# m3db/m3

Measured on AMD Instinct MI355X. Metric: datapoints/sec M3TSZ decode (1M series x 1440 pts) + HBM GB/s vs peak, higher is better.
Workload: dtype f64; 1 GPU; 1M series x 1440 pts batched M3TSZ decode, HBM-bandwidth microbench; nseries=1000000, npts=1440, data_detail=synthetic, parallelism=series-sharded x1 (no collectives)

## Files before the change

### m3_amd/csrc/m3tsz_kernels.hip

```cpp
#include <hip/hip_runtime.h>
#include <atomic>
#include <math.h>
#include <string.h>
#include <stdio.h>
#include "../../include/m3gpu.h"
#include "rollup_plan.h"


#define WAVE 64
#define WAVES_PER_BLOCK 4
#define BLOCK_THREADS (WAVE * WAVES_PER_BLOCK)

namespace m3 {

__device__ __constant__ int64_t UNIT_NS_D[9] = {
    0, 1000000000LL, 1000000LL, 1000LL, 1LL,
    60000000000LL, 3600000000000LL, 86400000000000LL, 31536000000000000LL};

#define MARKER_OPCODE 0x100ULL
#define MARKER_BITS 11
#define MARKER_EOS 0
#define MARKER_ANNOTATION 1
#define MARKER_TIMEUNIT 2

// ... 402 lines not shown
                prev_time_delta += dod;
                prev_time += prev_time_delta;
            }
        } else {
            *first = true;
            err = read_first_timestamp();
        }
        if (err) return err;
        if (tu_changed) { prev_time_delta = 0; tu_changed = false; }
        return 0;
    }

    __device__ __forceinline__ int read_full_float() {
        uint64_t vb;
        int err = r.read_bits(64, &vb);
        if (err) return err;
        prev_float_bits = vb;
        prev_xor = vb;
        return 0;
    }
    __device__ __forceinline__ int read_next_float() {
        uint64_t cb;
        int err = r.read_bits(1, &cb);
        if (err) return err;
        if (cb == 0) { prev_xor = 0; return 0; }
        uint64_t nxt;
        err = r.read_bits(1, &nxt);
        if (err) return err;
        cb = (cb << 1) | nxt;
        if (cb == 0x2) {
            uint32_t lead = prev_xor ? __builtin_clzll(prev_xor) : 64;
            uint32_t trail = prev_xor ? __builtin_ctzll(prev_xor) : 0;
            uint32_t nmean = 64 - lead - trail;
            uint64_t mb;
            err = r.read_bits(nmean, &mb);
            if (err) return err;
            prev_xor = mb << trail;
            prev_float_bits ^= prev_xor;
            return 0;
        }
        uint64_t lm;
        err = r.read_bits(12, &lm);
        if (err) return err;
        uint64_t lead = (lm & 4032) >> 6;
        uint64_t nmean = (lm & 63) + 1;
        uint64_t mb;
        err = r.read_bits((uint32_t)nmean, &mb);
        if (err) return err;
        uint64_t trail = 64 - lead - nmean;
        prev_xor = mb << trail;
        prev_float_bits ^= prev_xor;
        return 0;
    }

    __device__ __forceinline__ int read_int_sig_mult() {
        uint64_t b;
        int err = r.read_bits(1, &b);
        if (err) return err;
        if (b == 1) {
            err = r.read_bits(1, &b);
            if (err) return err;
            if (b == 0) sig = 0;
            else {
                uint64_t s;
                err = r.read_bits(NUM_SIG_BITS, &s);
                if (err) return err;
                sig = (uint8_t)s + 1;
            }
        }
        err = r.read_bits(1, &b);
        if (err) return err;
        if (b == 1) {
            uint64_t m;
            err = r.read_bits(NUM_MULT_BITS, &m);
            if (err) return err;
            mult = (uint8_t)m;
            if (mult > MAX_MULT) return M3GPU_SERIES_INVALID_MULT;
            mult_pow = exp10_sel(mult);
        }
        return 0;
    }
    __device__ __forceinline__ int read_int_val_diff() {
        if (sig == 64) {
            uint64_t sb;
            int err = r.read_bits(1, &sb);
            if (err) return err;
            double sgn = (sb == 1) ? 1.0 : -1.0;
            uint64_t bits;
            err = r.read_bits(sig, &bits);
            if (err) return err;
            int_val += sgn * (double)bits;
            return 0;
        }
        uint64_t bits;
        int err = r.read_bits((uint32_t)sig + 1, &bits);
        if (err) return err;
        double sgn = -1.0;
        if ((bits >> sig) == 1) { sgn = 1.0; bits ^= (1ULL << sig); }
        int_val += sgn * (double)bits;
        return 0;
    }

    __device__ __forceinline__ int read_first_value() {
        if (!int_optimized) return read_full_float();
        uint64_t b;
        int err = r.read_bits(1, &b);
        if (err) return err;
        if (b == 1) {
            err = read_full_float();
            if (err) return err;
            is_float = true;
            return 0;
        }
        err = read_int_sig_mult();
        if (err) return err;
        return read_int_val_diff();
    }
    __device__ __forceinline__ int read_next_value() {
        if (!int_optimized) return read_next_float();
        uint64_t b;
        int err = r.read_bits(1, &b);
        if (err) return err;
        if (b == 0) {
            err = r.read_bits(1, &b);
            if (err) return err;
            if (b == 1) return 0;
            err = r.read_bits(1, &b);
            if (err) return err;
            if (b == 1) {
                err = read_full_float();
                if (err) return err;
                is_float = true;
                return 0;
            }
            err = read_int_sig_mult();
            if (err) return err;
            err = read_int_val_diff();
            if (err) return err;
            is_float = false;
            return 0;
        }
        if (is_float) return read_next_float();
        return read_int_val_diff();
    }

    __device__ __forceinline__ int fused_xor(uint64_t w2, uint32_t pre) {
        if (!(w2 >> 63)) {
            r.consume(pre + 1);
            prev_xor = 0;
            return 0;
        }
        if ((w2 >> 62) == 0x2) {
            uint32_t lead = prev_xor ? __builtin_clzll(prev_xor) : 64;
            uint32_t trail = prev_xor ? __builtin_ctzll(prev_xor) : 0;
            uint32_t nmean = 64 - lead - trail;
            if (pre + 2 + nmean > 64) return -1000;
            uint64_t mb = nmean ? ((w2 << 2) >> (64 - nmean)) : 0;
            r.consume(pre + 2 + nmean);
            prev_xor = mb << trail;
            prev_float_bits ^= prev_xor;
            return 0;
        }
        uint64_t lead = (w2 >> 56) & 0x3f;
        uint64_t nmean = ((w2 >> 50) & 0x3f) + 1;
        r.consume(pre + 14);
        uint64_t mb;
        int err = r.read_bits((uint32_t)nmean, &mb);
        if (err) return -err;
        uint64_t trail = 64 - lead - nmean;
        prev_xor = mb << trail;
        prev_float_bits ^= prev_xor;
        return 0;
    }

    __device__ __forceinline__ int next_fused(int64_t* t, double* v) {
        if (tu_changed || !have_scheme || prev_time == 0 || r.bits_left < 64)
            return -1000;
        const uint64_t w = r.peek64();
        const uint64_t b0 = w >> 63;
        uint32_t tsbits = 1;
        int64_t dod = 0;
        if (b0) {
            const uint32_t L = (uint32_t)__builtin_clzll(~w);
            if (L >= 4 || (w >> 55) == MARKER_OPCODE)
                return -1000;
            const uint32_t vb = (0xC970u >> (L * 4)) & 0xFu;
            tsbits = L + 1 + vb;
            dod = sign_extend((w << (L + 1)) >> (64 - vb), vb) * unit_ns;
        }
        const uint64_t w2 = w << tsbits;

        if (int_optimized && !is_float) {
            const uint64_t v0 = w2 >> 63;
            const uint64_t v1 = (w2 >> 62) & 1;
            uint32_t nb;
            if (v0) {
                if (sig > 45u || tsbits + 2u + sig > 64u)
                    return -1000;
                nb = 2u + sig;
                const uint64_t field = (w2 << 1) >> (63u - sig);
                const uint64_t sbit = (field >> sig) & 1;
                const uint64_t mag = field ^ (sbit << sig);
                int_val += (sbit ? 1.0 : -1.0) * (double)mag;
            } else if (v1) {
                nb = 2;
            } else if ((w2 >> 61) & 1) {
                return -1000;
            } else {
                const uint64_t u = w2 << 3;
                uint8_t nsig = sig;
                uint32_t off;
                if (u >> 63) {
                    const uint64_t z = (u >> 62) & 1;
                    nsig = z ? (uint8_t)(((u >> 56) & 0x3f) + 1) : 0;
                    off = z ? 8u : 2u;
                } else {
                    off = 1u;
                }
                const uint64_t m = u << off;
                uint8_t nmult = mult;
                uint32_t moff;
                if (m >> 63) {
                    nmult = (uint8_t)((m >> 60) & 0x7);
                    moff = 4u;
                    if (nmult > MAX_MULT)
                        return -1000;
                } else {
                    moff = 1u;
                }
                if (nsig > 45u || tsbits + 3u + off + moff + 1u + nsig > 64u)
                    return -1000;
                const uint64_t f = m << moff;
                const uint64_t sbit = f >> 63;
                const uint64_t mag =
                    nsig ? ((f << 1) >> ((64u - nsig) & 63u)) : 0;
                int_val += (sbit ? 1.0 : -1.0) * (double)mag;
                sig = nsig;
                if (nmult != mult) { mult = nmult; mult_pow = exp10_sel(nmult); }
                nb = 3u + off + moff + 1u + nsig;
            }
            r.consume(tsbits + nb);
            prev_time_delta += dod;
            prev_time += prev_time_delta;
            *t = prev_time;
            double outv = int_val;
            if (mult != 0) outv = int_val / mult_pow;
            *v = outv;
            return 1;
        }
        int rx;
        if (!int_optimized) {
            rx = fused_xor(w2, tsbits);
        } else if (w2 >> 63) {
            rx = fused_xor(w2 << 1, tsbits + 1);
        } else if ((w2 >> 62) & 1) {
            r.consume(tsbits + 2);
            rx = 0;
        } else {
            return -1000;
        }
        if (rx == -1000) return -1000;
        if (rx) return rx;
        prev_time_delta += dod;
        prev_time += prev_time_delta;
        *t = prev_time;
        *v = bits2f(prev_float_bits);
        return 1;
    }

    __device__ __forceinline__ int next(int64_t* t, double* v) {
        if (done) return 0;
        int f = next_fused(t, v);
        if (f != -1000) {
            points += (f == 1);
            return f;
        }
        bool first;
        int err = read_timestamp(&first);
        if (err) return -err;
        if (done) return 0;
        err = first ? read_first_value() : read_next_value();
        if (err) return -err;
        *t = prev_time;
        if (!int_optimized || is_float) *v = bits2f(prev_float_bits);
        else if (mult != 0) *v = int_val / mult_pow;
        else *v = int_val;
        points++;
        return 1;
    }
    __device__ __forceinline__ double exp10_table(uint8_t m) {
        return exp10_sel(m);
    }
};

using Decoder = DecoderT<false>;
using RingDecoder = DecoderT<true>;


#define DEC_TILE 8
#ifndef RF_SPAN
#define RF_SPAN 2
#endif

__global__ void __launch_bounds__(BLOCK_THREADS, 4)
k_decode_batch(const uint8_t* __restrict__ blobs,
               const uint64_t* __restrict__ offsets,
               const uint32_t* __restrict__ lens,
               const int32_t* __restrict__ perm,
               uint32_t nseries, int int_optimized, uint8_t default_unit,
               int64_t* __restrict__ out_ts, double* __restrict__ out_vals,
               uint32_t* __restrict__ out_counts, int32_t* __restrict__ out_errs,
               uint32_t stride,
               uint8_t* __restrict__ out_ann, uint32_t ann_stride) {
    const uint32_t lane = threadIdx.x & (WAVE - 1);
    const uint32_t wave = __builtin_amdgcn_readfirstlane(threadIdx.x >> 6);
    const uint32_t slot = blockIdx.x * BLOCK_THREADS + wave * WAVE + lane;
    const uint32_t series = (perm && slot < nseries) ? (uint32_t)perm[slot] : slot;

    __shared__ uint64_t ring_all[WAVES_PER_BLOCK][WAVE][IN_STRIDE];
    __shared__ longlong2 tile_all[WAVES_PER_BLOCK][WAVE][DEC_TILE];
    uint64_t* ring = ring_all[wave][lane];
    longlong2 (*tile)[DEC_TILE] = tile_all[wave];

    const bool in_range = slot < nseries;
    RingDecoder d;
    d.init(blobs, in_range ? offsets[series] : 0, in_range ? lens[series] : 0,
           int_optimized != 0, default_unit, ring,
           (out_ann && in_range) ? out_ann + (uint64_t)series * ann_stride
                                 : nullptr,
           ann_stride);

    bool running = in_range;
    int err = 0;
    uint32_t cnt = 0;
    uint32_t k = 0;

    const bool discard = out_ts == nullptr;

    auto flush = [&](uint32_t base_pt) {
        if (discard) return;
        __builtin_amdgcn_wave_barrier();
        const uint32_t p = lane & (DEC_TILE - 1);
        const uint32_t r0 = lane / DEC_TILE;
        const uint32_t pt = base_pt + p;
        if (__all(cnt >= base_pt + DEC_TILE)) {
            for (uint32_t j = 0; j < DEC_TILE; j++) {
                uint32_t rr = r0 + j * (WAVE / DEC_TILE);
                uint32_t pc = p ^ (rr & 7);
                uint64_t row = (uint64_t)__shfl((int)series, (int)rr);
                longlong2 pr = tile[rr][pc];
                out_ts[row * stride + pt] = pr.x;
                out_vals[row * stride + pt] = __longlong_as_double(pr.y);
            }
        } else {
            for (uint32_t j = 0; j < DEC_TILE; j++) {
                uint32_t rr = r0 + j * (WAVE / DEC_TILE);
                uint32_t pc = p ^ (rr & 7);
                uint32_t cc = (uint32_t)__shfl((int)cnt, (int)rr);
                uint64_t row = (uint64_t)__shfl((int)series, (int)rr);
                if (pt < cc) {
                    longlong2 pr = tile[rr][pc];
                    out_ts[row * stride + pt] = pr.x;
                    out_vals[row * stride + pt] = __longlong_as_double(pr.y);
                }
            }
        }
        __builtin_amdgcn_wave_barrier();
    };

    auto step = [&](uint32_t j, bool check_cap) {
        if (running) {
            int64_t t;
            double v;
            int rstat = d.next(&t, &v);
            if (rstat <= 0) {
                err = -rstat;
                running = false;
            } else if (check_cap && cnt >= stride) {
                err = M3GPU_SERIES_CAPACITY;
                running = false;
            } else {
                if (!discard) {
                    uint32_t col = j ^ (lane & 7);
                    longlong2 pr;
                    pr.x = t;
                    pr.y = __double_as_longlong(v);
                    tile[lane][col] = pr;
                }
                cnt++;
            }
        }
    };

    while (__any(running)) {
        const bool check_cap = k + DEC_TILE > stride;
#pragma unroll 1
        for (uint32_t h = 0; h < DEC_TILE; h += RF_SPAN) {
            const RingPending pd = d.r.refill_issue(running);
#pragma unroll 1
            for (uint32_t j = h; j < h + RF_SPAN; j++) step(j, check_cap);
            d.r.refill_commit(pd);
        }
        flush(k);
        k += DEC_TILE;
    }

    if (in_range) {
        d.ann_finish(&err);
        out_counts[series] = cnt;
        out_errs[series] = err;
    }
}


struct BitWriter {
    uint64_t acc;
    uint32_t used;
    uint32_t nwords;
    uint64_t pend;
    uint64_t* out;
    uint32_t cap_words;
    int err;

    __device__ __forceinline__ void init(uint8_t* row, uint32_t cap_bytes) {
        acc = 0; used = 0; nwords = 0; pend = 0;
        out = (uint64_t*)row;
        cap_words = cap_bytes / 8;
        err = 0;
    }
    __device__ __forceinline__ void emit_word(uint64_t w) {
        if (nwords >= cap_words) { err = M3GPU_SERIES_CAPACITY; return; }
        if (nwords & 1) {
            ulonglong2 pr;
            pr.x = pend;
            pr.y = __builtin_bswap64(w);
            *(ulonglong2*)(out + nwords - 1) = pr;
        } else {
            pend = __builtin_bswap64(w);
        }
        nwords++;
    }
    __device__ __forceinline__ void write_bits(uint64_t v, uint32_t n) {
        if (n == 0 || err) return;
        v = (n >= 64) ? v : (v & ((1ULL << n) - 1));
        uint32_t space = 64 - used;
        if (n <= space) {
            acc |= v << (space - n);
            used += n;
            if (used == 64) { emit_word(acc); acc = 0; used = 0; }
        } else {
            uint32_t lo = n - space;
            acc |= v >> lo;
            emit_word(acc);
            acc = (lo >= 64) ? 0 : (v << (64 - lo));
            used = lo;
        }
    }
    __device__ __forceinline__ void write_bit(uint32_t b) { write_bits(b, 1); }
    __device__ __forceinline__ uint32_t finish() {
        if (nwords & 1) out[nwords - 1] = pend;
        uint32_t nbytes = nwords * 8;
        if (used > 0) {
            if (nwords >= cap_words) { err = M3GPU_SERIES_CAPACITY; return 0; }
            out[nwords] = __builtin_bswap64(acc);
            nbytes += (used + 7) / 8;
        }
        return nbytes;
    }
};

__device__ __forceinline__ double go_next_down(double x) {
    return __longlong_as_double(__double_as_longlong(x) - 1);
}
__device__ __forceinline__ double go_next_up(double x) {
    return __longlong_as_double(__double_as_longlong(x) + 1);
}

__device__ __forceinline__ int convert_to_int_float(double v, uint8_t cur_max_mult,
                                    double* out_val, uint8_t* out_mult, bool* out_is_float) {
    const double MAXINT = 9223372036854775808.0;
    if (cur_max_mult == 0 && v < MAXINT) {
        double i, r;
        r = go_modf(v, &i);
        if (r == 0) { *out_val = i; *out_mult = 0; *out_is_float = false; return 0; }
    }
    if (cur_max_mult > MAX_MULT) return M3GPU_SERIES_INVALID_MULT;
    double sign = 1.0;
    if (v < 0) sign = -1.0;
    for (uint8_t m = cur_max_mult; m <= MAX_MULT; m++) {
        double val = v * exp10_sel(m) * sign;
        if (val >= 1e13) break;
        double i, r;
        r = go_modf(val, &i);
        if (r == 0) { *out_val = sign * i; *out_mult = m; *out_is_float = false; return 0; }
        else if (r < 0.1) {
            if (go_next_down(val) <= i) { *out_val = sign * i; *out_mult = m; *out_is_float = false; return 0; }
        } else if (r > 0.9) {
            double nxt = i + 1;
            if (go_next_up(val) >= nxt) { *out_val = sign * nxt; *out_mult = m; *out_is_float = false; return 0; }
        }
    }
    *out_val = v; *out_mult = 0; *out_is_float = true;
    return 0;
}

#define XXH_P1 11400714785074694791ULL
#define XXH_P2 14029467366897019727ULL
#define XXH_P3 1609587929392839161ULL
#define XXH_P4 9650029242287828579ULL
#define XXH_P5 2870177450012600261ULL
#define XXH_EMPTY 0xEF46DB3751D8E999ULL

__device__ __forceinline__ uint64_t ld_le64(const uint8_t* p) {
    uint64_t v; __builtin_memcpy(&v, p, 8); return v;
}
__device__ __forceinline__ uint32_t ld_le32(const uint8_t* p) {
    uint32_t v; __builtin_memcpy(&v, p, 4); return v;
}
__device__ __forceinline__ uint64_t xxh_rotl(uint64_t x, uint32_t r) {
    return (x << r) | (x >> (64 - r));
}
__device__ __forceinline__ uint64_t xxh_round(uint64_t acc, uint64_t in) {
    return xxh_rotl(acc + in * XXH_P2, 31) * XXH_P1;
}
__device__ __forceinline__ uint64_t xxh_merge(uint64_t h, uint64_t v) {
    return (h ^ xxh_round(0, v)) * XXH_P1 + XXH_P4;
}
__device__ __noinline__ uint64_t xxh64(const uint8_t* p, uint32_t len) {
    const uint8_t* end = p + len;
    uint64_t h;
    if (len >= 32) {
        uint64_t v1 = XXH_P1 + XXH_P2, v2 = XXH_P2, v3 = 0, v4 = 0 - XXH_P1;
        do {
            v1 = xxh_round(v1, ld_le64(p));
            v2 = xxh_round(v2, ld_le64(p + 8));
            v3 = xxh_round(v3, ld_le64(p + 16));
            v4 = xxh_round(v4, ld_le64(p + 24));
            p += 32;
        } while (end - p >= 32);
        h = xxh_rotl(v1, 1) + xxh_rotl(v2, 7) + xxh_rotl(v3, 12) + xxh_rotl(v4, 18);
        h = xxh_merge(h, v1); h = xxh_merge(h, v2);
        h = xxh_merge(h, v3); h = xxh_merge(h, v4);
    } else {
        h = XXH_P5;
    }
    h += len;
    for (; end - p >= 8; p += 8)
        h = xxh_rotl(h ^ xxh_round(0, ld_le64(p)), 27) * XXH_P1 + XXH_P4;
    if (end - p >= 4) {
        h = xxh_rotl(h ^ (uint64_t)ld_le32(p) * XXH_P1, 23) * XXH_P2 + XXH_P3;
        p += 4;
    }
    for (; p < end; p++)
        h = xxh_rotl(h ^ (uint64_t)*p * XXH_P5, 11) * XXH_P1;
    h ^= h >> 33; h *= XXH_P2; h ^= h >> 29; h *= XXH_P3; h ^= h >> 32;
    return h;
}

struct Encoder {
    BitWriter w;
    int64_t unit_ns;
    int64_t prev_time, prev_time_delta;
    uint64_t prev_xor, prev_float_bits;
    double int_val;
    uint8_t time_unit, max_mult;
    uint8_t num_sig_state, cur_highest_lower_sig, num_lower_sig;
    bool has_written_first, is_float, int_optimized;
    uint32_t num_encoded;
    uint64_t prev_ann_checksum;

    __device__ __forceinline__ void init(uint8_t* row, uint32_t cap_bytes,
                         int64_t start_ns, bool intopt, uint8_t default_unit) {
        w.init(row, cap_bytes);
        prev_time = start_ns;
        prev_time_delta = 0;
        prev_ann_checksum = XXH_EMPTY;
        prev_xor = 0; prev_float_bits = 0;
        int_val = 0;
        unit_ns = unit_valid(default_unit) ? UNIT_NS_D[default_unit] : 0;
        time_unit = (unit_valid(default_unit) && unit_ns != 0 &&
                     start_ns % unit_ns == 0) ? default_unit : 0;
        max_mult = 0;
        num_sig_state = 0; cur_highest_lower_sig = 0; num_lower_sig = 0;
        has_written_first = false; is_float = false;
        int_optimized = intopt;
        num_encoded = 0;
    }

    __device__ __forceinline__ void write_marker(uint32_t marker) {
        w.write_bits(MARKER_OPCODE, 9);
        w.write_bits(marker, 2);
    }

    __device__ __forceinline__ int64_t div_unit(int64_t x) const {
        switch (unit_ns) {
        case 1LL: return x;
        case 1000LL: return x / 1000LL;
        case 1000000LL: return x / 1000000LL;
        case 1000000000LL: return x / 1000000000LL;
        default: return x / unit_ns;
        }
    }

    __device__ __forceinline__ int write_dod_unchanged(int64_t prev_delta, int64_t cur_delta, uint8_t unit) {
        if (!unit_valid(unit)) return M3GPU_SERIES_NO_SCHEME;
        int64_t dod = div_unit(cur_delta - prev_delta);
        if (unit == 1 || unit == 2) {
            if ((int64_t)(int32_t)dod != dod) return M3GPU_SERIES_DOD_OVERFLOW;
        }
        int dbits = scheme_default_bits(unit);
        if (!dbits) return M3GPU_SERIES_NO_SCHEME;
        if (dod == 0) { w.write_bits(0, 1); return 0; }
        const uint64_t m = (uint64_t)(dod < 0 ? ~dod : dod);
        const uint32_t nb = (m ? 64u - (uint32_t)__builtin_clzll(m) : 0u) + 1u;
        if (nb <= 12u) {
            const uint32_t sel = (nb <= 7u) ? 0u : (nb <= 9u) ? 1u : 2u;
            const uint32_t opc = (sel == 0) ? 0x2u : (sel == 1) ? 0x6u : 0xeu;
            const uint32_t vb = (sel == 0) ? 7u : (sel == 1) ? 9u : 12u;
            w.write_bits(opc, sel + 2u);
            w.write_bits((uint64_t)dod, vb);
            return 0;
        }
        w.write_bits(0xf, 4);
        w.write_bits((uint64_t)dod, dbits);
        return 0;
    }

    __device__ __forceinline__ void write_annotation(const uint8_t* ant, uint32_t len) {
        uint64_t checksum = xxh64(ant, len);
        if (checksum == prev_ann_checksum) return;
        write_marker(MARKER_ANNOTATION);
        uint64_t ux = (uint64_t)(len - 1) << 1;
        for (; ux >= 0x80; ux >>= 7) w.write_bits((ux & 0x7f) | 0x80, 8);
        w.write_bits(ux, 8);
        uint32_t i = 0;
        for (; len - i >= 8; i += 8)
            w.write_bits(__builtin_bswap64(ld_le64(ant + i)), 64);
        for (; i < len; i++) w.write_bits(ant[i], 8);
        prev_ann_checksum = checksum;
    }

    __device__ __forceinline__ int write_time(int64_t cur_time, uint8_t unit) {
        if (!has_written_first) {
            w.write_bits((uint64_t)prev_time, 64);
            has_written_first = true;
        }
        bool tu_changed = false;
        if (unit_valid(unit) && unit != time_unit) {
            write_marker(MARKER_TIMEUNIT);
            w.write_bits(unit, 8);
            time_unit = unit;
            unit_ns = UNIT_NS_D[unit];
            tu_changed = true;
        }
        int64_t time_delta = cur_time - prev_time;
        prev_time = cur_time;
        if (tu_changed) {
            w.write_bits((uint64_t)(time_delta - prev_time_delta), 64);
            prev_time_delta = 0;
            return 0;
        }
        int err = write_dod_unchanged(prev_time_delta, time_delta, unit);
        prev_time_delta = time_delta;
        return err;
    }

    __device__ __forceinline__ void write_full_float(uint64_t val) {
        prev_float_bits = val;
        prev_xor = val;
        w.write_bits(val, 64);
    }
    __device__ __forceinline__ void write_xor(uint64_t cur_xor) {
        if (cur_xor == 0) { w.write_bits(0, 1); return; }
        uint32_t pl = prev_xor ? __builtin_clzll(prev_xor) : 64;
        uint32_t pt = prev_xor ? __builtin_ctzll(prev_xor) : 0;
        uint32_t cl = __builtin_clzll(cur_xor);
        uint32_t ct = __builtin_ctzll(cur_xor);
        if (cl >= pl && ct >= pt) {
            w.write_bits(0x2, 2);
            w.write_bits(cur_xor >> pt, 64 - pl - pt);
            return;
        }
        w.write_bits(0x3, 2);
        w.write_bits(cl, 6);
        uint32_t nmean = 64 - cl - ct;
        w.write_bits(nmean - 1, 6);
// ... 1748 lines not shown
```

Measured before the change: 98.12 billion datapoints/sec.

## Widen decode output flush to 16-byte nontemporal stores with new LDS swizzle

Reworks the per-tile flush of decoded timestamps and values so each lane writes two adjacent points per store (dwordx4) instead of one 8-byte store, using a new swizzle so paired columns sit next to each other in shared memory. Output stores default to nontemporal hints so the write-once result streams don't pollute cache. Falls back to the old narrow path when stride or pointer alignment does not allow 16-byte stores. The change targets store instruction count and write efficiency on the HBM-bound output, and adds branching and swizzle complexity.

```diff
diff --git a/m3_amd/csrc/m3tsz_kernels.hip b/m3_amd/csrc/m3tsz_kernels.hip
--- a/m3_amd/csrc/m3tsz_kernels.hip
+++ b/m3_amd/csrc/m3tsz_kernels.hip
@@ -728,6 +728,49 @@
 #define RF_SPAN 2
 #endif
 
+#ifndef OUT_POLICY
+#define OUT_POLICY 1
+#endif
+
+#ifndef FLUSH_WIDE
+#define FLUSH_WIDE 1
+#endif
+
+typedef long long dec_ll2 __attribute__((ext_vector_type(2)));
+
+template <typename T>
+__device__ __forceinline__ void out_st8(T* p, long long x) {
+    static_assert(sizeof(T) == 8, "8-byte element");
+#if OUT_POLICY == 2
+    __hip_atomic_store((long long*)p, x, __ATOMIC_RELAXED,
+                       __HIP_MEMORY_SCOPE_AGENT);
+#elif OUT_POLICY == 1
+    __builtin_nontemporal_store(x, (long long*)p);
+#else
+    *(long long*)p = x;
+#endif
+}
+
+template <typename T>
+__device__ __forceinline__ void out_st16(T* p, long long x0, long long x1) {
+    static_assert(sizeof(T) == 8, "8-byte element");
+    dec_ll2 v;
+    v.x = x0;
+    v.y = x1;
+#if OUT_POLICY == 2
+    asm volatile("global_store_dwordx4 %0, %1, off sc1\n\ts_nop 1"
+                 :: "v"(p), "v"(v));
+#elif OUT_POLICY == 1
+    __builtin_nontemporal_store(v, (dec_ll2*)p);
+#else
+    *(dec_ll2*)p = v;
+#endif
+}
+
+__device__ __forceinline__ uint32_t dec_swz(uint32_t r) {
+    return ((r & 1) << 2) | (r & 2) | ((r >> 2) & 1);
+}
+
 __global__ void __launch_bounds__(BLOCK_THREADS, 4)
 k_decode_batch(const uint8_t* __restrict__ blobs,
                const uint64_t* __restrict__ offsets,
@@ -762,35 +805,65 @@
     uint32_t k = 0;
 
     const bool discard = out_ts == nullptr;
-
+    const bool wide = FLUSH_WIDE && !discard && !(stride & 1) &&
+        !(((uintptr_t)out_ts | (uintptr_t)out_vals) & 15);
+    const uint32_t swz = dec_swz(lane & 7);
+
+    auto flush_wide = [&](uint32_t base_pt) {
+        const uint32_t q = lane & 3;
+        const uint32_t r0 = lane >> 2;
+        const uint32_t pt = base_pt + 2 * q;
+        const uint32_t pc = (2 * q) ^ dec_swz(r0 & 7);
+        if (__all(cnt >= base_pt + DEC_TILE)) {
+            for (uint32_t j = 0; j < DEC_TILE / 2; j++) {
+                uint32_t rr = r0 + j * (WAVE / 4);
+                uint64_t row = (uint64_t)__shfl((int)series, (int)rr);
+                longlong2 p0 = tile[rr][pc];
+                longlong2 p1 = tile[rr][pc ^ 1];
+                out_st16(out_ts + row * stride + pt, p0.x, p1.x);
+                out_st16(out_vals + row * stride + pt, p0.y, p1.y);
+            }
+        } else {
+            for (uint32_t j = 0; j < DEC_TILE / 2; j++) {
+                uint32_t rr = r0 + j * (WAVE / 4);
+                uint32_t cc = (uint32_t)__shfl((int)cnt, (int)rr);
+                uint64_t row = (uint64_t)__shfl((int)series, (int)rr);
+                if (pt < cc) {
+                    longlong2 p0 = tile[rr][pc];
+                    if (pt + 1 < cc) {
+                        longlong2 p1 = tile[rr][pc ^ 1];
+                        out_st16(out_ts + row * stride + pt, p0.x, p1.x);
+                        out_st16(out_vals + row * stride + pt, p0.y, p1.y);
+                    } else {
+                        out_st8(out_ts + row * stride + pt, p0.x);
+                        out_st8(out_vals + row * stride + pt, p0.y);
+                    }
+                }
+            }
+        }
+    };
+    auto flush_narrow = [&](uint32_t base_pt) {
+        const uint32_t p = lane & (DEC_TILE - 1);
+        const uint32_t r0 = lane / DEC_TILE;
+        const uint32_t pt = base_pt + p;
+        const uint32_t pc = p ^ dec_swz(r0 & 7);
+        const bool full = __all(cnt >= base_pt + DEC_TILE);
+        for (uint32_t j = 0; j < DEC_TILE; j++) {
+            uint32_t rr = r0 + j * (WAVE / DEC_TILE);
+            uint32_t cc = (uint32_t)__shfl((int)cnt, (int)rr);
+            uint64_t row = (uint64_t)__shfl((int)series, (int)rr);
+            if (full || pt < cc) {
+                longlong2 pr = tile[rr][pc];
+                out_st8(out_ts + row * stride + pt, pr.x);
+                out_st8(out_vals + row * stride + pt, pr.y);
+            }
+        }
+    };
     auto flush = [&](uint32_t base_pt) {
         if (discard) return;
         __builtin_amdgcn_wave_barrier();
-        const uint32_t p = lane & (DEC_TILE - 1);
-        const uint32_t r0 = lane / DEC_TILE;
-        const uint32_t pt = base_pt + p;
-        if (__all(cnt >= base_pt + DEC_TILE)) {
-            for (uint32_t j = 0; j < DEC_TILE; j++) {
-                uint32_t rr = r0 + j * (WAVE / DEC_TILE);
-                uint32_t pc = p ^ (rr & 7);
-                uint64_t row = (uint64_t)__shfl((int)series, (int)rr);
-                longlong2 pr = tile[rr][pc];
-                out_ts[row * stride + pt] = pr.x;
-                out_vals[row * stride + pt] = __longlong_as_double(pr.y);
-            }
-        } else {
-            for (uint32_t j = 0; j < DEC_TILE; j++) {
-                uint32_t rr = r0 + j * (WAVE / DEC_TILE);
-                uint32_t pc = p ^ (rr & 7);
-                uint32_t cc = (uint32_t)__shfl((int)cnt, (int)rr);
-                uint64_t row = (uint64_t)__shfl((int)series, (int)rr);
-                if (pt < cc) {
-                    longlong2 pr = tile[rr][pc];
-                    out_ts[row * stride + pt] = pr.x;
-                    out_vals[row * stride + pt] = __longlong_as_double(pr.y);
-                }
-            }
-        }
+        if (wide) flush_wide(base_pt);
+        else flush_narrow(base_pt);
         __builtin_amdgcn_wave_barrier();
     };
 
@@ -807,7 +880,7 @@
                 running = false;
             } else {
                 if (!discard) {
-                    uint32_t col = j ^ (lane & 7);
+                    uint32_t col = j ^ swz;
                     longlong2 pr;
                     pr.x = t;
                     pr.y = __double_as_longlong(v);
```

Result: faster. 100.9 billion datapoints/sec, median of 6 (+2.9%).
